# samson6460/tf2_YOLO

Hardware: AMD Instinct MI355X
Metric: images/sec training YOLOv3 416x416 bs=32/GPU (higher is better)
Workload: dtype f32-storage/fp16x2-mfma

## Files before the change

### include/yolo_hip.h

```cpp
#ifndef YOLO_HIP_H_
#define YOLO_HIP_H_

#include <stddef.h>
#include <stdint.h>

#ifdef __cplusplus
extern "C" {
#endif

typedef enum yolo_status {
  YOLO_OK = 0,
  YOLO_ERR_INVALID_ARG = -1,
  YOLO_ERR_LAUNCH = -2,
  YOLO_ERR_WORKSPACE = -3
} yolo_status;

enum { YOLO_ACT_LINEAR = 0, YOLO_ACT_LEAKY = 1, YOLO_ACT_MISH = 2 };
enum { YOLO_HEAD_V3 = 3, YOLO_HEAD_V2 = 2, YOLO_HEAD_V1 = 1, YOLO_HEAD_V4 = 4 };
enum { YOLO_NMS_HARD = 1, YOLO_NMS_SOFT = 2, YOLO_NMS_DIOU = 3 };

const char* yolo_last_error(void);
int yolo_abi_version(void);
int yolo_device_available(void);
int yolo_mfma_probe(const void* operands_f16, float* sink, int workgroups, int iters, double* flops_host, void* stream);

enum { YOLO_OPT_CONV_WIN = 0, YOLO_OPT_STAMPS = 1, YOLO_OPT_CONV_SK = 2, YOLO_OPT_CONV_PATCH = 5, YOLO_OPT_WGRAD_WIN = 6,
       YOLO_OPT_NMS_WALK = 7 ,
       YOLO_OPT_AB = 8  };
int yolo_set_option(int key, int value);
size_t yolo_conv_workspace_bytes(void);
int yolo_set_conv_workspace(void* p, size_t bytes, void* stream);
int yolo_set_debug_buffer(void* p, size_t bytes);

typedef struct yolo_conv_desc {
  int N, H, W, Cin;
  int Cout, kh, kw;
  int Ho, Wo;
  int sh, sw;
  int pad_t, pad_l;
} yolo_conv_desc;

#define YOLO_BN_STAT_SLOTS 64
// ... 246 lines not shown
```

### tf2_yolo_amd/csrc/conv.hip

```cpp
#include "conv_args.hpp"
#include <cstdlib>
#include <type_traits>

namespace yolo {

template <int BM, int BN, int WGM, int WGN, bool FLAT>
__global__ __launch_bounds__(256) void gather_conv_kernel(const GatherConvArgs a) {
  constexpr int BK = 32;
  constexpr int LD = BK + 4;
  constexpr int TM = BM / WGM / 32;
  constexpr int TN = BN / WGN / 32;
  constexpr int AR = BM / 32;
  constexpr int BR = BN / 32;
  static_assert(WGM * WGN == 4, "4 waves per block");
  static_assert(TM >= 1 && TN >= 1, "wave tile");

  extern __shared__ __attribute__((aligned(16))) float smem[];
  constexpr int BUF = (BM + BN) * LD;

  const int tid = threadIdx.x;
  const int lane = tid & 63;
  const int wave = tid >> 6;
  const int wm = wave / WGN, wn = wave % WGN;

// ... 1026 lines not shown
  int cap;
  unsigned* aux;
  int nslots;
};
static void set_bnred(GatherConvArgs& a, const BnRedArgs* b) {
  if (b == nullptr) return;
  a.bwd_y = b->y; a.bwd_scale = b->scale; a.bwd_shift = b->shift; a.bwd_mean = b->mean; a.bwd_invstd = b->invstd;
  a.bwd_act = b->act; a.bwd_part = b->part; a.bwd_cap = b->cap; a.bwd_aux = b->aux;
}

static int dgrad_impl(const yolo_conv_desc* d, const float* dy, const float* wT, float* dx, int accumulate,
                      void* stream, bool planes, BnRedArgs* bnred = nullptr) {
  if (int rc = validate_desc(d)) return rc;
  YOLO_REQUIRE(dy && wT && dx, "conv_dgrad: null pointer");
  const bool flat = (d->Cout % 32) != 0;
  YOLO_REQUIRE(!flat || (d->kh == 1 && d->kw == 1 && d->sh == 1 && d->sw == 1),
               "conv_dgrad: Cout %% 32 != 0 only supported for 1x1 stride-1 (head) convs");
  static const bool fuse_classes = env_int("YOLO_DGRAD_CLASSES", 1) != 0;
  if (planes && fuse_classes && d->sh * d->sw > 1 && d->sh * d->sw <= 4) {
    GatherConvArgs a{};
    a.src = dy;
    a.wgt = wT;
    a.dst = dx;
    a.N = d->N; a.Hs = d->Ho; a.Ws = d->Wo; a.Cs = d->Cout;
    a.sy = 1; a.sx = 1;
    a.Hd = d->H; a.Wd = d->W; a.Cd = d->Cin;
    a.osy = d->sh; a.osx = d->sw;
    a.Cout = d->Cin;
    a.ldw = d->kh * d->kw * d->Cout;
    a.accumulate = accumulate;
    a.kw = 1;
    int nt = 0, nc = 0;
    bool ok = true;
// ... 196 lines not shown
```

### tf2_yolo_amd/csrc/conv_args.hpp

```cpp
#pragma once
#include "common.hpp"

namespace yolo {

constexpr int MAX_TAPS = 49;

struct Tap {
  int oy, ox, woff;
};

struct ClassGeom {
  long long M;
  int Hg, Wg, ooy, oox, tap0, ntaps;
};

struct GatherConvArgs {
  const float* src;
  const float* wgt;
  const float* bias;
  float* dst;
  double* stats;
  unsigned* absmax;
  long long M;
  int N, Hs, Ws, Cs;
// ... 20 lines not shown
  const float* pl_pred;
  const unsigned* pl_in_bound;
  const unsigned* pl_res_bound;
  int pl_in_n, pl_res_n;
  unsigned* pl_out_words;
  float* head_y;
  const float* head_anchors;
  int head_A, head_C;
  int sk_grid;
  int tile_order;
  float* sk_slabs;
  unsigned* sk_tickets;
  int split_parts;
  int ncls;
  ClassGeom cls[4];
  unsigned long long* stamps;
  const float* bwd_y;
  const float* bwd_scale;
  const float* bwd_shift;
  const float* bwd_mean;
  const float* bwd_invstd;
  float* bwd_part;
  unsigned* bwd_aux;
  int bwd_act;
  int bwd_nslots;
  int bwd_cap;
  Tap taps[MAX_TAPS];
};

#define YOLO_BNRED_CHECK(a)                                                                                          \
// ... 40 lines not shown
                               void* planes, float* dst32, float* out_bound, hipStream_t st,
                               const int* bound_words = nullptr, const int* upsample = nullptr, int H = 0, int W = 0);
int launch_split_planes_padded(const float* x, long long rows, int Csrc, int C, void* planes, hipStream_t st);
int launch_split_planes_batch(const void* jobs, int njobs, long long total_blocks, hipStream_t st);
int launch_filter_transpose_batch(const void* jobs, int njobs, long long total_blocks, hipStream_t st);
int launch_gather_planes(GatherConvArgs& a, hipStream_t st);
bool conv_small_supported(const GatherConvArgs& a);
bool conv_small_head_supported(const GatherConvArgs& a);
int launch_conv_small(GatherConvArgs& a, hipStream_t st, int* nwg);
bool gather_planes_supported(const GatherConvArgs& a);
int conv_split_parts(const GatherConvArgs& a, long long nb, int bm, int min_cb, int idle_div);
int launch_split_reduce(GatherConvArgs& a, int bm, hipStream_t st);
float* conv_split_slabs();
int launch_conv_win(GatherConvArgs& a, int variant, hipStream_t st);
bool conv_win_supported(const GatherConvArgs& a);
enum { OPT_CONV_WIN = 0, OPT_STAMPS = 1, OPT_CONV_SK = 2, OPT_DBG = 3, OPT_TILE_ORDER = 4, OPT_CONV_PATCH = 5, OPT_WGRAD_WIN = 6, OPT_NMS_WALK = 7, OPT_EXP = 8, OPT_COUNT = 16 };
int set_conv_workspace(void* p, size_t bytes, hipStream_t st);
extern void* g_dbg_buf;
extern size_t g_dbg_bytes;
extern int g_opt[OPT_COUNT];
void init_options();
int launch_wgrad_planes(WgradArgs& a, hipStream_t st);
bool wgrad_planes_supported(const WgradArgs& a);
int launch_wgrad_win(WgradArgs& a, hipStream_t st);
bool wgrad_win_supported(const WgradArgs& a);
constexpr size_t WGRAD_WS_COLSUM_BYTES = 1 << 20;
void* wgrad_workspace(size_t* bytes);
bool stem_fwd_supported(const yolo_conv_desc* d);
struct StemEpiArgs {
  const float* scale;
  const float* shift;
// ... 23 lines not shown
```

### tf2_yolo_amd/csrc/conv_planes.hip

```cpp
#include "planes_epilogue.hpp"
#include <algorithm>
#include <cstdlib>
#include <type_traits>

namespace yolo {

__global__ __launch_bounds__(256) void planes_amax_kernel(const float* __restrict__ x, long long n4,
                                                         unsigned* __restrict__ header) {
  float m = 0.f;
  for (long long i = (long long)blockIdx.x * 256 + threadIdx.x; i < n4; i += (long long)gridDim.x * 256) {
    const f32x4 v = reinterpret_cast<const f32x4*>(x)[i];
    m = fmaxf(fmaxf(m, fmaxf(fabsf(v[0]), fabsf(v[1]))), fmaxf(fabsf(v[2]), fabsf(v[3])));
  }
#pragma unroll
  for (int o = 32; o > 0; o >>= 1) m = fmaxf(m, __shfl_xor(m, o, 64));
  __shared__ float wmax[4];
  if ((threadIdx.x & 63) == 0) wmax[threadIdx.x >> 6] = m;
  __syncthreads();
  if (threadIdx.x == 0) {
    m = fmaxf(fmaxf(wmax[0], wmax[1]), fmaxf(wmax[2], wmax[3]));
    if (__builtin_bit_cast(unsigned, m) > *reinterpret_cast<volatile unsigned*>(header))
      atomicMax(header, __builtin_bit_cast(unsigned, m));
  }
}
// ... 216 lines not shown
      if (g * 8 + 4 + j < Csrc) v1[j] = p[g * 8 + 4 + j];
    }
  }
  const Planes8 s = split8(v0, v1, sc);
  unsigned char* o = out + planes_unit_offset(row, g, C);
  *reinterpret_cast<u32x4*>(o) = s.h;
  *reinterpret_cast<u32x4*>(o + 512) = s.l;
}

constexpr int PF_KO_MASK = 31;
constexpr int PF_SPLIT = 32;
constexpr int PF_MULTI = 64;
constexpr int PF_DEEP1 = 128;
constexpr int PF_DEEP2 = 256;
constexpr int PF_BNRED = 512;
template <int BM, int BN, int WGM, int WGN, int FORM = 0>
__global__ __launch_bounds__(64 * WGM * WGN, (WGM * WGN >= 4 ? 2 : 1)) void gather_conv_planes_kernel(const GatherConvArgs a) {
  constexpr int NW = WGM * WGN;
  constexpr int TM = BM / WGM / 32;
  constexpr int TN = BN / WGN / 32;
  constexpr int RBA = BM / 32, RBB = BN / 32;
  constexpr int LPW = (RBA + RBB + NW - 1) / NW;
  static_assert(LPW <= 4, "loader layout: slot s = wave + i*NW loads A block s, or B block (s - RBA) % RBB");
  constexpr int ND = PL_PLANES * LPW;
  constexpr int STAGE_BYTES = (RBA + RBB) * PL_PLANES * 1024;
  constexpr int NBUF = 3 + ((FORM >> 7) & 3);

  extern __shared__ __attribute__((aligned(16))) unsigned char smem[];
  const unsigned lds_base = (unsigned)(size_t)smem;

  const int tid = threadIdx.x;
  const int lane = tid & 63;
  const int wave = __builtin_amdgcn_readfirstlane(tid >> 6);
  const int wm = wave / WGN, wn = wave % WGN;

  constexpr bool SPLIT = (FORM & PF_SPLIT) != 0;
  const int SP = SPLIT ? a.split_parts : 1;
  const int part = SPLIT ? (int)blockIdx.x / a.nblocks : 0;
  const int tile = xcd_remap(SPLIT ? (int)blockIdx.x - part * a.nblocks : (int)blockIdx.x, a.nblocks);
  constexpr bool MULTI = (FORM & PF_MULTI) != 0;
  constexpr bool BNRED = (FORM & PF_BNRED) != 0;
  const int tile_n = tile % a.tiles_n;
  const int cls = MULTI ? (tile / a.tiles_n) % a.ncls : 0;
  const int tile_m = MULTI ? tile / (a.tiles_n * a.ncls) : tile / a.tiles_n;
  const long long m0 = (long long)tile_m * BM;
  const int n0 = tile_n * BN;
  const EpiGeom G = MULTI ? EpiGeom{a.cls[cls].M, a.cls[cls].Hg, a.cls[cls].Wg, a.cls[cls].ooy, a.cls[cls].oox, 0, 0, 0,
                                    tile_m * a.ncls + cls + 1}
                          : epi_geom_of(a);
  const int tap0 = MULTI ? a.cls[cls].tap0 : 0;
  const int ntaps = MULTI ? a.cls[cls].ntaps : a.ntaps;
  if (MULTI && m0 >= G.M) {
    if (a.bwd_y != nullptr)
      for (int c = tid; c < BN; c += 64 * NW)
        if (n0 + c < a.Cout) {
          a.bwd_part[((long long)(G.slot1 - 1) * 2 + 0) * a.Cout + n0 + c] = 0.f;
// ... 18 lines not shown
#pragma unroll
  for (int i = 0; i < LPW; ++i) {
    const int slot = wave + i * NW;
    isA[i] = slot < RBA;
    const int rb = isA[i] ? slot : (slot - RBA) % RBB;
    nimg[i] = 0; ys0[i] = -(1 << 28); xs0[i] = 0; rowbaseB[i] = 0;
    if (isA[i]) {
      const long long m = m0 + rb * 32 + r;
      if (m < G.M) {
        nimg[i] = (int)(m / HgWg);
        const int rem = (int)(m - (long long)nimg[i] * HgWg);
        const int y = rem / G.Wg;
        ys0[i] = y * a.sy;
        xs0[i] = (rem - y * G.Wg) * a.sx;
      }
    } else {
      const int co = n0 + rb * 32 + r;
      const unsigned blk = co < a.Cout ? (unsigned)(co >> 4) : (unsigned)a.zero_blk_wgt;
      rowbaseB[i] = blk * blkstrideB + (co < a.Cout ? (co & 15) * 16 : 0) + hf * 256;
    }
    lds_mine[i] = lds_base + ((isA[i] ? 0 : RBA) + rb) * PL_PLANES * 1024;
    ld_voff[i] = 0; ld_soff[i] = 0;
  }

  int ld_tap = 0, ld_kk = 0, ld_cb = cb_lo;
  auto loader_tap = [&]() {
#pragma unroll
    for (int i = 0; i < LPW; ++i) {
      if (ld_cb >= cpt) {
        ld_voff[i] = isA[i] ? (unsigned)a.zero_blk_src * blkstrideA : (unsigned)a.zero_blk_wgt * blkstrideB;
        ld_soff[i] = 0;
      } else if (isA[i]) {
        const int ys = ys0[i] + a.taps[tap0 + ld_tap].oy, xs = xs0[i] + a.taps[tap0 + ld_tap].ox;
        const bool ok = ((unsigned)ys < (unsigned)a.Hs) && ((unsigned)xs < (unsigned)a.Ws);
        const int pix = (nimg[i] * a.Hs + ys) * a.Ws + xs;
        ld_voff[i] = (ok ? ((unsigned)pix >> 4) : (unsigned)a.zero_blk_src) * blkstrideA + (ok ? (pix & 15) * 16 : 0) + hf * 256;
        ld_soff[i] = (unsigned)ld_cb * PL_RECORD;
      } else {
        ld_voff[i] = rowbaseB[i];
        ld_soff[i] = (unsigned)((a.taps[tap0 + ld_tap].woff >> 4) + ld_cb) * PL_RECORD;
      }
    }
  };
  auto loader_next = [&]() {
#pragma unroll
    for (int i = 0; i < LPW; ++i) ld_soff[i] += PL_RECORD;
    const int kc_cur = (cpt - ld_cb < a.kc) ? (cpt - ld_cb) : a.kc;
    if (++ld_kk >= kc_cur) {
      ld_kk = 0;
      if (++ld_tap == ntaps) {
        ld_tap = 0;
        ld_cb += a.kc;
// ... 24 lines not shown

  f16x8 fa[2][PL_PLANES][TM], fb[2][PL_PLANES][TN];
  auto read_frags = [&](int buf, auto SET) {
    constexpr int S = decltype(SET)::value;
    const unsigned char* sb = smem + buf * STAGE_BYTES + lane * 16;
#pragma unroll
    for (int p = 0; p < PL_PLANES; ++p) {
#pragma unroll
      for (int i = 0; i < TM; ++i)
        fa[S][p][i] = *reinterpret_cast<const f16x8*>(sb + ((wm * TM + i) * PL_PLANES + p) * 1024);
#pragma unroll
      for (int j = 0; j < TN; ++j)
        fb[S][p][j] = *reinterpret_cast<const f16x8*>(sb + ((RBA + wn * TN + j) * PL_PLANES + p) * 1024);
    }
  };
  auto mfma_stage = [&](auto SET, int wbuf) {
    constexpr int S = decltype(SET)::value;
    constexpr int NM = TM * TN * 3;
#pragma unroll
    for (int q = 0; q < 3; ++q) {
      const int pa = (q == 0) ? 1 : 0;
      const int pb = (q == 1) ? 1 : 0;
#pragma unroll
      for (int i = 0; i < TM; ++i)
#pragma unroll
        for (int j = 0; j < TN; ++j) {
          if constexpr (!(FORM & 8)) acc[i][j] = __builtin_amdgcn_mfma_f32_32x32x16_f16(fa[S][pa][i], fb[S][pb][j], acc[i][j], 0, 0, 0);
          const int idx = (q * TM + i) * TN + j;
#pragma unroll
          for (int d = 0; d < ND; ++d)
            if (idx == (((d + 1) * NM) / (ND + 1) > 0 ? ((d + 1) * NM) / (ND + 1) - 1 : 0)) {
              __builtin_amdgcn_sched_barrier(0);
              if constexpr (!(FORM & 1)) issue_plane(d, wbuf);
              __builtin_amdgcn_sched_barrier(0);
            }
        }
    }
    loader_next();
  };

  using S0 = std::integral_constant<int, 0>;
  using S1 = std::integral_constant<int, 1>;
// ... 19 lines not shown
    for (; kt + 1 < nk; kt += 2) {
      step(rbuf, wbuf, S0{}, S1{});
      rbuf = (rbuf + 1 == NBUF) ? 0 : rbuf + 1;
      wbuf = (wbuf + 1 == NBUF) ? 0 : wbuf + 1;
      step(rbuf, wbuf, S1{}, S0{});
      rbuf = (rbuf + 1 == NBUF) ? 0 : rbuf + 1;
      wbuf = (wbuf + 1 == NBUF) ? 0 : wbuf + 1;
    }
    if (kt < nk) step(rbuf, wbuf, S0{}, S1{});
  }
  asm volatile("s_waitcnt vmcnt(0)" ::: "memory");
  __syncthreads();

  if constexpr (SPLIT)
    store_split_slab<TM, TN>(a, acc, BM * BN * 4, tile * SP + part, wave, lane);
  else if constexpr (MULTI)
    planes_epilogue<BM, BN, WGM, WGN, NBUF * STAGE_BYTES, 0, NoStamp, false, BNRED>(a, acc, smem, m0, n0, tile_m, wm, wn, lane, tid, NoStamp(), &G);
  else
    planes_epilogue<BM, BN, WGM, WGN, NBUF * STAGE_BYTES, (FORM & PF_KO_MASK), NoStamp, false, BNRED>(a, acc, smem, m0, n0, tile_m, wm, wn, lane, tid);
}

template <int BM, int BN, int WGM, int WGN, int FORM = 0>
static int launch_planes(GatherConvArgs& a, hipStream_t st) {
  const long long tiles_m = (a.M + BM - 1) / BM;
  a.tiles_n = (a.Cout + BN - 1) / BN;
  const long long nb = tiles_m * a.tiles_n;
  if (nb <= 0 || nb > 0x7fffffffLL) {
    set_error("conv(planes): bad grid %lld", nb);
    return YOLO_ERR_INVALID_ARG;
  }
// ... 23 lines not shown
  a.bwd_nslots = (int)tiles_m;
  YOLO_BNRED_CHECK(a)
  constexpr auto plain = &gather_conv_planes_kernel<BM, BN, WGM, WGN, FORM>;
  a.split_parts = 1;
  if constexpr (BM == 128 && BN == 128 && WGM == 2 && WGN == 2 && FORM == 0) {
    const int min_cb = a.ntaps >= 8 ? 1 : (8 + a.ntaps - 1) / a.ntaps;
    a.split_parts = conv_split_parts(a, nb, BM, min_cb, 4);
    if (a.split_parts > 1) {
      a.sk_slabs = conv_split_slabs();
      if (int rc = launch_lds<gather_conv_planes_kernel<BM, BN, WGM, WGN, PF_SPLIT>, lds>(
              dim3((unsigned)(nb * a.split_parts)), block, st, a, "gather_conv_planes_kernel(split)"))
        return rc;
      return launch_split_reduce(a, BM, st);
    }
  }
  if constexpr ((FORM & ~(PF_DEEP1 | PF_DEEP2)) == 0) {
    if (a.bwd_y != nullptr)
      return launch_lds<gather_conv_planes_kernel<BM, BN, WGM, WGN, FORM | PF_BNRED>, lds>(dim3((unsigned)nb), block, st, a,
                                                                                          "gather_conv_planes_kernel(bn reduce)");
  } else if (a.bwd_y != nullptr) {
    set_error("conv(planes): this diagnostic instantiation has no fused BatchNorm-backward reduction");
    return YOLO_ERR_INVALID_ARG;
  }
  return launch_lds<plain, lds>(dim3((unsigned)nb), block, st, a, "gather_conv_planes_kernel");
}

long long planes_bytes(long long rows, int C) { return planes_body_bytes(rows, C) + PL_HEADER; }

bool gather_planes_supported(const GatherConvArgs& a) { return (a.Cs % 16) == 0 && a.Cout >= 32; }

int launch_gather_planes(GatherConvArgs& a, hipStream_t st) {
  const long long rowsA = (long long)a.N * a.Hs * a.Ws;
  const long long bytesA = planes_bytes(rowsA, a.Cs), bytesB = planes_bytes(a.Cout, a.ldw);
  if (bytesA >= (1LL << 32) || bytesB >= (1LL << 32)) {
    set_error("conv(planes): operand planes exceed 4 GiB (%lld, %lld bytes)", bytesA, bytesB);
    return YOLO_ERR_INVALID_ARG;
  }
  a.src_bytes = (unsigned)bytesA;
  a.wgt_bytes = (unsigned)bytesB;
  a.zero_blk_src = (int)((rowsA + 15) / 16);
  a.zero_blk_wgt = (a.Cout + 15) / 16;
  static const int nt = env_int("YOLO_NT_STORE", 1);
  a.nt_store = nt;
  static const int vecst = env_int("YOLO_VEC_STORE", 1);
  a.vec_store = vecst;
  static const int dbg = env_int("YOLO_PLANES_DBG", 0);
  a.dbg = dbg;
  static const int kc_env = env_int("YOLO_PLANES_KC", 0);
  a.kc = kc_env > 0 ? kc_env : (a.Cs >> 4);
  if (a.kc > (a.Cs >> 4)) a.kc = a.Cs >> 4;
  init_options();
  if (g_opt[OPT_CONV_WIN] != 0 && a.ncls <= 1) {
    const int rc = launch_conv_win(a, g_opt[OPT_CONV_WIN], st);
    if (rc <= 0) return rc;
  }
  static const int deep_env = env_int("YOLO_PLANES_DEEP", -1);
  const int deep = deep_env >= 0 ? deep_env : (a.Cout <= 64 ? 1 : 2);
  if (deep && a.ntaps == 1 && a.ncls <= 1) {
    if (a.Cout <= 32) return deep == 1 ? launch_planes<128, 32, 4, 1, PF_DEEP1>(a, st) : launch_planes<128, 32, 4, 1, PF_DEEP2>(a, st);
    if (a.Cout <= 64) return deep == 1 ? launch_planes<128, 64, 4, 2, PF_DEEP1>(a, st) : launch_planes<128, 64, 4, 2, PF_DEEP2>(a, st);
  }
  if (a.Cout <= 32) return launch_planes<128, 32, 4, 1>(a, st);
  if (a.Cout <= 64) return launch_planes<128, 64, 4, 2>(a, st);
  static const int narrow_below = env_int("YOLO_PLANES_NARROW_BELOW", 0);
  if (((a.M + 127) / 128) * ((a.Cout + 127) / 128) < narrow_below) return launch_planes<128, 64, 4, 2>(a, st);
  static const int waves_env = env_int("YOLO_PLANES_WAVES", 0);
// ... 284 lines not shown
```

### tf2_yolo_amd/csrc/planes_epilogue.hpp

```cpp
#pragma once
#include "planes.hpp"
#include "act.hpp"

namespace yolo {

struct NoStamp {
  __device__ __forceinline__ void operator()(int) const {}
};

struct EpiGeom {
  long long M;
  int Hg, Wg, ooy, oox;
  int pn, py0, px0;
  int slot1;
};
__device__ __forceinline__ EpiGeom epi_geom_of(const GatherConvArgs& a) {
  return EpiGeom{a.M, a.Hg, a.Wg, a.ooy, a.oox, 0, 0, 0, 0};
}

template <int TM, int TN>
__device__ __forceinline__ void store_split_slab(const GatherConvArgs& a, f32x16 (&acc)[TM][TN], const int slab_bytes,
                                                 const int slab, const int wave, const int lane) {
  unsigned char* mine = reinterpret_cast<unsigned char*>(a.sk_slabs) + (size_t)slab * slab_bytes;
  const __amdgpu_buffer_rsrc_t rs = __builtin_amdgcn_make_buffer_rsrc(mine, 0, slab_bytes, 0x00020000);
#pragma unroll
  for (int i = 0; i < TM; ++i)
#pragma unroll
    for (int j = 0; j < TN; ++j)
#pragma unroll
      for (int q4 = 0; q4 < 4; ++q4) {
        const f32x4 f = {acc[i][j][4 * q4], acc[i][j][4 * q4 + 1], acc[i][j][4 * q4 + 2], acc[i][j][4 * q4 + 3]};
        __builtin_amdgcn_raw_buffer_store_b128(__builtin_bit_cast(u32x4, f), rs,
                                               (((wave * TM + i) * TN + j) * 4 + q4) * 1024 + lane * 16, 0, 0);
      }
}

template <int BM, int BN, int WGM, int WGN, int LDS_BYTES, int DBG = 0, class STAMP = NoStamp, bool PATCH = false, bool BNRED = false>
__device__ __forceinline__ void planes_epilogue(const GatherConvArgs& a, f32x16 (&acc)[BM / WGM / 32][BN / WGN / 32],
                                                unsigned char* smem, const long long m0, const int n0, const int tile_m,
                                                const int wm, const int wn, const int lane, const int tid,
                                                const STAMP& stampf = STAMP(), const EpiGeom* geom = nullptr) {
  const EpiGeom G = geom != nullptr ? *geom : epi_geom_of(a);
  constexpr int NT = 64 * WGM * WGN;
  constexpr int NW = WGM * WGN;
  constexpr int TM = BM / WGM / 32;
  constexpr int TN = BN / WGN / 32;
  const int wave = wm * WGN + wn;
  float* smf = reinterpret_cast<float*>(smem);
  long long* rowoff = reinterpret_cast<long long*>(smf);
  const bool dense = a.osy == 1 && a.osx == 1 && G.ooy == 0 && G.oox == 0 && a.Hd == G.Hg && a.Wd == G.Wg;
  {
    const int HgWg = G.Hg * G.Wg;
    for (int rr = tid; rr < BM; rr += NT) {
      const long long m = m0 + rr;
      long long off = -1;
      if constexpr (PATCH) {
        const int y = G.py0 + (rr >> 4), x = G.px0 + (rr & 15);
        if (y < G.Hg && x < G.Wg) off = (((long long)G.pn * a.Hd + y) * a.Wd + x) * a.Cd;
      } else if (m < G.M) {
        if (dense) {
          off = m * a.Cd;
        } else {
          const int n = (int)(m / HgWg);
          const int rem = (int)(m - (long long)n * HgWg);
          const int y = rem / G.Wg;
          const int x = rem - y * G.Wg;
          off = (((long long)n * a.Hd + (y * a.osy + G.ooy)) * a.Wd + (x * a.osx + G.oox)) * a.Cd;
        }
      }
      rowoff[rr] = off;
    }
  }
  __syncthreads();
  stampf(0);

  const float unscale =
      reinterpret_cast<const float*>(reinterpret_cast<const unsigned char*>(a.src) + a.src_bytes - PL_HEADER)[2] *
      reinterpret_cast<const float*>(reinterpret_cast<const unsigned char*>(a.wgt) + a.wgt_bytes - PL_HEADER)[2];
  float* sred = smf + 2 * BM;
  float csum[TN], csq[TN], cmx[TN];
#pragma unroll
  for (int j = 0; j < TN; ++j) csum[j] = csq[j] = cmx[j] = 0.f;
  [[maybe_unused]] float bs1[TN], bs2[TN];
#pragma unroll
  for (int j = 0; j < TN; ++j) bs1[j] = bs2[j] = 0.f;
  asm volatile("" ::"v"(unscale));
  stampf(1);
  const int rows_valid = PATCH ? BM : ((G.M - m0 < (long long)BM) ? (int)(G.M - m0) : BM);
  const bool want_stats = a.stats != nullptr || a.absmax != nullptr;
  [[maybe_unused]] unsigned long long rowmask = ~0ull;
  if constexpr (PATCH) {
    static_assert(BM / WGM / 32 <= 4, "row mask: at most 4 row blocks per wave");
    rowmask = 0;
    if (want_stats) {
#pragma unroll
      for (int i = 0; i < BM / WGM / 32; ++i)
#pragma unroll
        for (int q = 0; q < 16; ++q)
          if (rowoff[(wm * (BM / WGM / 32) + i) * 32 + (q & 3) + 8 * (q >> 2) + 4 * (lane >> 5)] >= 0)
            rowmask |= 1ull << (i * 16 + q);
    }
  }
  const bool bnred = BNRED && a.bwd_y != nullptr && a.stats == nullptr;
  float bn_mx = 0.f;
  constexpr int WCOLS = TN * 32;
  constexpr int TLD = WCOLS + 4;
  constexpr int FIXED = 2 * BM + WGM * BN * 3;
  constexpr int RP = ((FIXED + NW * 32 * TLD) * 4 <= LDS_BYTES) ? 32 : 16;
  constexpr bool VEC_OK = (FIXED + NW * RP * TLD) * 4 <= LDS_BYTES && (RP * WCOLS / 4) % 64 == 0;
  const bool vec = VEC_OK && a.vec_store && (a.Cout & 3) == 0 && (a.Cd & 3) == 0 && !(a.accumulate && a.stats != nullptr) &&
                   (DBG & 16) == 0;
  if constexpr (VEC_OK) {
  if (vec) {
    float* strip = smf + FIXED + wave * (RP * TLD);
    constexpr int C4 = WCOLS / 4;
    constexpr int ITER = RP * C4 / 64;
    static_assert(64 % C4 == 0, "store loop: a lane keeps its four columns");
    const int bcol = n0 + wn * WCOLS + (lane % C4) * 4;
    f32x4 b_sc = {0.f, 0.f, 0.f, 0.f}, b_sh = b_sc, b_mu = b_sc, b_iv = b_sc, b_s1 = b_sc, b_s2 = b_sc;
    constexpr int NPASS = TM * (32 / RP);
    constexpr bool PRE_OLD = TM * TN <= 2;
    [[maybe_unused]] f32x4 ypre[BNRED ? NPASS : 1][BNRED ? ITER : 1];
    [[maybe_unused]] f32x4 opre[BNRED && PRE_OLD ? NPASS : 1][BNRED && PRE_OLD ? ITER : 1];
    if constexpr (BNRED)
// ... 98 lines not shown
                const f32x4 yv = ypre[ps][h0 + k];
#pragma unroll
                for (int e = 0; e < 4; ++e) {
                  const float dz = v[e] * act_grad(fmaf(b_sc[e], yv[e], b_sh[e]), a.bwd_act);
                  b_s1[e] += dz;
                  b_s2[e] = fmaf(dz, (yv[e] - b_mu[e]) * b_iv[e], b_s2[e]);
                  bn_mx = fmaxf(bn_mx, fabsf(dz));
                }
              }
            }
          }
          }
        } else {
        long long offs[ITER];
        f32x4 vv[ITER];
#pragma unroll
        for (int it = 0; it < ITER; ++it) {
          const int idx = lane + it * 64;
          const int rl = idx / C4, c4 = idx - rl * C4;
          offs[it] = rowoff[row0 + rl];
          vv[it] = *reinterpret_cast<const f32x4*>(strip + rl * TLD + c4 * 4);
        }
#pragma unroll
        for (int it = 0; it < ITER; ++it) {
          const int idx = lane + it * 64;
          const int c4 = idx % C4;
          const int col = n0 + wn * WCOLS + c4 * 4;
          if (offs[it] >= 0 && col < a.Cout) {
            f32x4* p = reinterpret_cast<f32x4*>(a.dst + offs[it] + col);
            f32x4 v = vv[it];
            if (a.epi_res != nullptr) v += *reinterpret_cast<const f32x4*>(a.epi_res + offs[it] + col);
            if (a.accumulate) v += *p;
            if (a.nt_store) __builtin_nontemporal_store(v, p); else *p = v;
          }
        }
        }
        asm volatile("s_waitcnt lgkmcnt(0)" ::: "memory");
      }
    }
    if (bnred) {
#pragma unroll
      for (int o = C4; o < 64; o <<= 1)
#pragma unroll
        for (int e = 0; e < 4; ++e) {
          b_s1[e] += __shfl_xor(b_s1[e], o, 64);
          b_s2[e] += __shfl_xor(b_s2[e], o, 64);
// ... 7 lines not shown
      }
    }
    stampf(2);
  }
  }
  if (!vec) {
#pragma unroll
    for (int i = 0; i < TM; ++i) {
      long long offs[16];
#pragma unroll
      for (int q = 0; q < 16; ++q) offs[q] = rowoff[(wm * TM + i) * 32 + (q & 3) + 8 * (q >> 2) + 4 * (lane >> 5)];
#pragma unroll
      for (int j = 0; j < TN; ++j) {
        const int col = n0 + (wn * TN + j) * 32 + (lane & 31);
        const bool cok = col < a.Cout;
        const float bv = (a.bias != nullptr && cok) ? a.bias[col] : 0.f;
        const float esc = (a.epi_scale != nullptr && cok) ? a.epi_scale[col] : 1.f;
        const float esh = (a.epi_scale != nullptr && cok) ? a.epi_shift[col] : 0.f;
        const float rsc = (bnred && cok) ? a.bwd_scale[col] : 0.f, rsh = (bnred && cok) ? a.bwd_shift[col] : 0.f;
        const float rmu = (bnred && cok) ? a.bwd_mean[col] : 0.f, riv = (bnred && cok) ? a.bwd_invstd[col] : 0.f;
#pragma unroll
        for (int q = 0; q < 16; ++q) {
          const bool ok = cok && offs[q] >= 0;
          float v = fmaf(acc[i][j][q], unscale, bv);
          if (a.epi_scale != nullptr) v = act_fwd(fmaf(esc, v, esh), a.epi_act);
          const float vstat = v;
          if (ok) {
            if (a.epi_res != nullptr) v += a.epi_res[offs[q] + col];
            if (a.accumulate) v += a.dst[offs[q] + col];
            if constexpr ((DBG & 16) != 0) { if (v == 1234.5678f) a.dst[offs[q] + col] = v; }
            else if (a.nt_store && !bnred) __builtin_nontemporal_store(v, &a.dst[offs[q] + col]); else a.dst[offs[q] + col] = v;
            if (bnred) {
              const float yv = a.bwd_y[offs[q] + col];
              const float dz = v * act_grad(fmaf(rsc, yv, rsh), a.bwd_act);
              bs1[j] += dz;
              bs2[j] = fmaf(dz, (yv - rmu) * riv, bs2[j]);
              bn_mx = fmaxf(bn_mx, fabsf(dz));
            }
          }
          const float vm = ok ? (a.epi_scale != nullptr ? vstat : v) : 0.f;
          csum[j] += vm;
          csq[j] = fmaf(vm, vm, csq[j]);
          cmx[j] = fmaxf(cmx[j], fabsf(vm));
        }
      }
    }
  }
  if (bnred) {
// ... 72 lines not shown
```

### tf2_yolo_amd/csrc/runtime.hip

```cpp
#include "conv_args.hpp"
#include <cstdlib>
#include <cstring>

namespace yolo {

static thread_local char g_err[512] = "";

void set_error(const char* fmt, ...) {
  va_list ap;
  va_start(ap, fmt);
  vsnprintf(g_err, sizeof(g_err), fmt, ap);
  va_end(ap);
}

int g_opt[OPT_COUNT];
void* g_dbg_buf = nullptr;
size_t g_dbg_bytes = 0;
static void options_from_env() {
  for (int i = 0; i < OPT_COUNT; ++i) g_opt[i] = 0;
  g_opt[OPT_CONV_WIN] = env_int("YOLO_CONV_WIN", 1);
  g_opt[OPT_CONV_SK] = env_int("YOLO_CONV_SK", 1);
  g_opt[OPT_CONV_PATCH] = env_int("YOLO_CONV_PATCH", 1);
  g_opt[OPT_WGRAD_WIN] = env_int("YOLO_WGRAD_WIN", 1);
  g_opt[OPT_NMS_WALK] = env_int("YOLO_NMS_WALK", 0);
  g_opt[OPT_EXP] = env_int("YOLO_EXP", 0);
}
void init_options() {
  static bool done = false;
  if (done) return;
  done = true;
  options_from_env();
}

}

extern "C" int yolo_set_option(int key, int value) {
  yolo::init_options();
  if (key == -1) {
    yolo::options_from_env();
    return YOLO_OK;
// ... 62 lines not shown
```

### tf2_yolo_amd/ops.py

```python
import ctypes
from ctypes import byref, c_void_p

import torch

from . import _lib
from . import tape as _tape
from ._lib import ConvDesc, LossCfg, YoloHipError, check

BN_EPS = 1e-3
BN_MOMENTUM = 0.99
BN_STAT_SLOTS = 64
BN_RED_SLOTS = 512
SPLIT_BATCH_UNITS = 4


class KernelTimer:

    def __init__(self):
        self.pending = []

    def bracket(self, name, flops, launches, fn, layer=None):
        s, e = torch.cuda.Event(enable_timing=True), torch.cuda.Event(enable_timing=True)
        s.record()
        fn()
# ... 80 lines not shown
        if CONV_PATCH == 2 or ((narrow or ws > 64) and tiles >= 256):
            return "conv_patch_planes_kernel<%s>" % ("256,64" if narrow else "128,128")
    if win is not None and CONV_WIN and cout >= 128:
        ws, m = win[:2]
        wgm = CONV_WIN if CONV_WIN in (2, 4) else (0 if ws > 64 else 2)
        if wgm:
            return "conv_win_planes_kernel<%d,128>" % (64 * wgm)
    if cout <= 32:
        return "gather_conv_planes_kernel<128,32,4,1>"
    if cout <= 64:
        return "gather_conv_planes_kernel<128,64,4,2>"
    waves8 = _PLANES_WAVES == 8 or (_PLANES_WAVES == 0 and k1)
    return "gather_conv_planes_kernel<128,128,%s>" % ("4,2" if waves8 else "2,2")


def _win_key(d, hs, ws, cs):
    if d.kh == 3 and d.kw == 3 and d.sh == 1 and d.sw == 1 and d.pad_t == 1 and d.pad_l == 1 and cs % 16 == 0 \
            and d.H == d.Ho and d.W == d.Wo:
        return (ws, d.N * hs * ws, hs, d.N)
    return None


def _gather_variant(cout, flat, m=None):
    bn = 32 if cout <= 32 else (64 if cout <= 64 else 128)
    bm = 128
    if bn == 128 and not flat and m is not None and ((m + 127) // 128) * ((cout + 127) // 128) <= 512:
        bm = 64
    if CONV_MODE == "split" and not flat and cout > 32:
        waves = {(128, 64): "2,2", (64, 128): "1,4", (128, 128): "4,2"}[(bm, bn)]
        return f"gather_conv_split_kernel<{bm},{bn},{waves}>"
    return f"gather_conv_kernel<{bm},{bn}{',flat' if flat else ''}>"


OPT_CONV_WIN = 0
OPT_CONV_SK = 2
OPT_CONV_PATCH = 5
OPT_WGRAD_WIN = 6
OPT_NMS_WALK = 7
_CONV_WS = None


def ensure_conv_workspace():
    global _CONV_WS
    if _CONV_WS is not None and _CONV_WS.device.index != torch.cuda.current_device():
        raise YoloHipError(f"libyolo_hip.so was initialised on cuda:{_CONV_WS.device.index} and cannot also serve "
                           f"cuda:{torch.cuda.current_device()}: start one process per GPU")
    if _CONV_WS is None:
        lib = _lib.load()
        n = int(lib.yolo_conv_workspace_bytes())
        _CONV_WS = torch.empty(n, dtype=torch.uint8, device="cuda")
        check(lib.yolo_set_conv_workspace(_p(_CONV_WS), n, _stream()), "yolo_set_conv_workspace")
    return _CONV_WS

# ... 58 lines not shown
                              "will run them one after the other (create_side_streams() earlier, or raise GPU_MAX_HW_QUEUES)")
            _SIDE_STREAMS[(dev, role)] = st
            _first_use(st, dev)
    return {role: _SIDE_STREAMS[(dev, role)] for role in ("wgrad", "comm")}


def concurrent_stream(role, beside=None, device=None):
    st = create_side_streams(device)[role]
    want = torch.cuda.current_device() if device is None else torch.device(device).index
    if want is not None and st.device.index != want:
        raise YoloHipError(f"side stream of role {role!r} lives on cuda:{st.device.index}, not on cuda:{want}")
    return st


def set_option(key, value):
    global WGRAD_WIN
    check(_lib.load().yolo_set_option(int(key), int(value)), "yolo_set_option")
    if int(key) == OPT_WGRAD_WIN:
        WGRAD_WIN = int(value)


def reset_options():
    global WGRAD_WIN
    check(_lib.load().yolo_set_option(-1, 0), "yolo_set_option")
    WGRAD_WIN = int(_os.environ.get("YOLO_WGRAD_WIN", "1"))


def _stream():
    return c_void_p(torch.cuda.current_stream().cuda_stream)


def _p(t):
    if t is None:
        return c_void_p(0)
    if _tape.ACTIVE is not None:
        _tape.ACTIVE.keep.append(t)
    return c_void_p(t.data_ptr())


def _chk_f32(*ts):
# ... 313 lines not shown
        if (b.y.numel() != dx.numel() or min(t.numel() for t in (b.scale, b.shift, b.mean, b.invstd)) < d.Cin
                or b.partials.numel() < b.cap * 2 * d.Cin or b.aux is None or b.aux.numel() < 68):
            raise YoloHipError("conv2d_dgrad_planes: the fused reduction's buffers do not match the descriptor")
    def run():
        if bnred is None:
            check(_lib.load().yolo_conv2d_dgrad_planes(byref(d), _p(dyp), _p(wTp), _p(dx), int(bool(accumulate)), _stream()),
                  "yolo_conv2d_dgrad_planes")
            return
        n = ctypes.c_int(0)
        check(_lib.load().yolo_conv2d_dgrad_planes_bnred(byref(d), _p(dyp), _p(wTp), _p(dx), int(bool(accumulate)), _p(b.y),
                                                         _p(b.scale), _p(b.shift), _p(b.mean), _p(b.invstd), int(b.act),
                                                         _p(b.partials), int(b.cap), _p(b.aux), byref(n), _stream()),
              "yolo_conv2d_dgrad_planes_bnred")
        b.nslots = n.value
    if TIMER is not None:
        TIMER.bracket(_planes_variant(d.Cin, _win_key(d, d.Ho, d.Wo, d.Cout), d.kh * d.kw == 1 and d.sh * d.sw == 1), _conv_flops(d), 1, run,
                      _layer_key(d, "dgrad"))
    else:
        run()
    return dx


def conv2d_wgrad_planes(d, xp, dyp, dw, dy=None, dbias=None):
    _chk_f32(dw, dy, dbias)
    if dw.numel() != d.Cout * d.kh * d.kw * d.Cin:
        raise YoloHipError("conv2d_wgrad_planes: dw size does not match the descriptor")
    if xp.numel() < planes_bytes(d.N * d.H * d.W, d.Cin) or dyp.numel() < planes_bytes(d.N * d.Ho * d.Wo, d.Cout):
        raise YoloHipError("conv2d_wgrad_planes: planes buffers do not match the descriptor")
    def run():
        check(_lib.load().yolo_conv2d_wgrad_planes(byref(d), _p(xp), _p(dyp), _p(dw), _stream()),
              "yolo_conv2d_wgrad_planes")
    if TIMER is not None:
# ... 578 lines not shown
```

Baseline: 1081.

## Pack four output-parity classes into one 128-column tile for Cin=32 dgrad

For data-gradient convolutions with only 32 input channels, the four 2x2 output-parity classes are stacked as four 32-wide column groups of one 128-column MFMA tile. Each class gets its own weight-offset table per source tap, and the epilogue uses four row-offset tables to scatter results back to the interleaved output pixels. This is meant to fill the otherwise mostly-empty N dimension of the tile and read dy once for all classes. A default skip mask avoids MFMAs on class/tap pairs with no weight. The cost is extra epilogue address work and extra LDS for the tables.

```diff
diff --git a/include/yolo_hip.h b/include/yolo_hip.h
--- a/include/yolo_hip.h
+++ b/include/yolo_hip.h
@@ -26,6 +26,7 @@
 
 enum { YOLO_OPT_CONV_WIN = 0, YOLO_OPT_STAMPS = 1, YOLO_OPT_CONV_SK = 2, YOLO_OPT_CONV_PATCH = 5, YOLO_OPT_WGRAD_WIN = 6,
        YOLO_OPT_NMS_WALK = 7 ,
+       YOLO_OPT_DGRAD_COLS = 9,
        YOLO_OPT_AB = 8  };
 int yolo_set_option(int key, int value);
 size_t yolo_conv_workspace_bytes(void);
diff --git a/tf2_yolo_amd/csrc/conv.hip b/tf2_yolo_amd/csrc/conv.hip
--- a/tf2_yolo_amd/csrc/conv.hip
+++ b/tf2_yolo_amd/csrc/conv.hip
@@ -1,4 +1,5 @@
 #include "conv_args.hpp"
+#include "dgrad_cols_plan.hpp"
 #include <cstdlib>
 #include <type_traits>
 
@@ -1064,9 +1065,41 @@
   if (int rc = validate_desc(d)) return rc;
   YOLO_REQUIRE(dy && wT && dx, "conv_dgrad: null pointer");
   const bool flat = (d->Cout % 32) != 0;
-  YOLO_REQUIRE(!flat || (d->kh == 1 && d->kw == 1 && d->sh == 1 && d->sw == 1),
+  YOLO_REQUIRE(planes || !flat || (d->kh == 1 && d->kw == 1 && d->sh == 1 && d->sw == 1),
                "conv_dgrad: Cout %% 32 != 0 only supported for 1x1 stride-1 (head) convs");
   static const bool fuse_classes = env_int("YOLO_DGRAD_CLASSES", 1) != 0;
+  init_options();
+  if (planes && bnred == nullptr && g_opt[OPT_DGRAD_COLS] != 0 && d->Cin == 32 && d->Cout % 16 == 0 && d->kh * d->kw <= 9) {
+    const int o = g_opt[OPT_DGRAD_COLS];
+    const bool strided = d->sh * d->sw > 1;
+    const bool want = strided ? (o & 1) != 0 : (d->kh * d->kw > 1 ? (o & 2) != 0 : (o & 8) != 0);
+    DgradColsPlan pl;
+    if (want && dgrad_cols_plan(d, &pl)) {
+      GatherConvArgs a{};
+      a.src = dy;
+      a.wgt = wT;
+      a.dst = dx;
+      a.N = d->N; a.Hs = d->Ho; a.Ws = d->Wo; a.Cs = d->Cout;
+      a.Hg = pl.Hg; a.Wg = pl.Wg;
+      a.sy = pl.step_y; a.sx = pl.step_x;
+      a.Hd = d->H; a.Wd = d->W; a.Cd = d->Cin;
+      a.osy = 2; a.osx = 2;
+      a.cols = d->Cin;
+      a.cols_dense = (o & 4) != 0;
+      a.Cout = DGC_CLASSES * d->Cin;
+      a.ldw = d->kh * d->kw * d->Cout;
+      a.accumulate = accumulate;
+      a.kw = 1;
+      a.M = (long long)d->N * pl.Hg * pl.Wg;
+      a.ntaps = pl.ntaps;
+      for (int t = 0; t < pl.ntaps; ++t) {
+        a.taps[t] = Tap{pl.oy[t], pl.ox[t], 0};
+        for (int q = 0; q < DGC_CLASSES; ++q) a.cwoff[t][q] = pl.woff[t][q];
+      }
+      a.cmask = pl.used;
+      return launch_gather_planes(a, as_stream(stream));
+    }
+  }
   if (planes && fuse_classes && d->sh * d->sw > 1 && d->sh * d->sw <= 4) {
     GatherConvArgs a{};
     a.src = dy;
diff --git a/tf2_yolo_amd/csrc/conv_args.hpp b/tf2_yolo_amd/csrc/conv_args.hpp
--- a/tf2_yolo_amd/csrc/conv_args.hpp
+++ b/tf2_yolo_amd/csrc/conv_args.hpp
@@ -58,6 +58,9 @@
   int split_parts;
   int ncls;
   ClassGeom cls[4];
+  int cols, cols_dense;
+  int cwoff[16][4];
+  unsigned long long cmask;
   unsigned long long* stamps;
   const float* bwd_y;
   const float* bwd_scale;
@@ -128,7 +131,7 @@
 float* conv_split_slabs();
 int launch_conv_win(GatherConvArgs& a, int variant, hipStream_t st);
 bool conv_win_supported(const GatherConvArgs& a);
-enum { OPT_CONV_WIN = 0, OPT_STAMPS = 1, OPT_CONV_SK = 2, OPT_DBG = 3, OPT_TILE_ORDER = 4, OPT_CONV_PATCH = 5, OPT_WGRAD_WIN = 6, OPT_NMS_WALK = 7, OPT_EXP = 8, OPT_COUNT = 16 };
+enum { OPT_CONV_WIN = 0, OPT_STAMPS = 1, OPT_CONV_SK = 2, OPT_DBG = 3, OPT_TILE_ORDER = 4, OPT_CONV_PATCH = 5, OPT_WGRAD_WIN = 6, OPT_NMS_WALK = 7, OPT_EXP = 8, OPT_DGRAD_COLS = 9, OPT_COUNT = 16 };
 int set_conv_workspace(void* p, size_t bytes, hipStream_t st);
 extern void* g_dbg_buf;
 extern size_t g_dbg_bytes;
diff --git a/tf2_yolo_amd/csrc/conv_planes.hip b/tf2_yolo_amd/csrc/conv_planes.hip
--- a/tf2_yolo_amd/csrc/conv_planes.hip
+++ b/tf2_yolo_amd/csrc/conv_planes.hip
@@ -254,6 +254,8 @@
 constexpr int PF_DEEP1 = 128;
 constexpr int PF_DEEP2 = 256;
 constexpr int PF_BNRED = 512;
+constexpr int PF_COLS = 1024;
+constexpr int PF_COLSKIP = 2048;
 template <int BM, int BN, int WGM, int WGN, int FORM = 0>
 __global__ __launch_bounds__(64 * WGM * WGN, (WGM * WGN >= 4 ? 2 : 1)) void gather_conv_planes_kernel(const GatherConvArgs a) {
   constexpr int NW = WGM * WGN;
@@ -280,6 +282,9 @@
   const int tile = xcd_remap(SPLIT ? (int)blockIdx.x - part * a.nblocks : (int)blockIdx.x, a.nblocks);
   constexpr bool MULTI = (FORM & PF_MULTI) != 0;
   constexpr bool BNRED = (FORM & PF_BNRED) != 0;
+  constexpr bool COLS = (FORM & PF_COLS) != 0;
+  constexpr bool COLSKIP = (FORM & PF_COLSKIP) != 0;
+  static_assert(!COLS || (BN == 128 && RBB == 4 && !MULTI && !SPLIT && !BNRED), "class columns: one 128-column tile, four classes");
   const int tile_n = tile % a.tiles_n;
   const int cls = MULTI ? (tile / a.tiles_n) % a.ncls : 0;
   const int tile_m = MULTI ? tile / (a.tiles_n * a.ncls) : tile / a.tiles_n;
@@ -328,6 +333,8 @@
         ys0[i] = y * a.sy;
         xs0[i] = (rem - y * G.Wg) * a.sx;
       }
+    } else if constexpr (COLS) {
+      rowbaseB[i] = (unsigned)(r >> 4) * blkstrideB + (r & 15) * 16 + hf * 256;
     } else {
       const int co = n0 + rb * 32 + r;
       const unsigned blk = co < a.Cout ? (unsigned)(co >> 4) : (unsigned)a.zero_blk_wgt;
@@ -350,6 +357,10 @@
         const int pix = (nimg[i] * a.Hs + ys) * a.Ws + xs;
         ld_voff[i] = (ok ? ((unsigned)pix >> 4) : (unsigned)a.zero_blk_src) * blkstrideA + (ok ? (pix & 15) * 16 : 0) + hf * 256;
         ld_soff[i] = (unsigned)ld_cb * PL_RECORD;
+      } else if constexpr (COLS) {
+        const int wo = a.cwoff[ld_tap][(wave + i * NW - RBA) % RBB];
+        ld_voff[i] = wo >= 0 ? rowbaseB[i] : (unsigned)a.zero_blk_wgt * blkstrideB;
+        ld_soff[i] = wo >= 0 ? (unsigned)((wo >> 4) + ld_cb) * PL_RECORD : 0u;
       } else {
         ld_voff[i] = rowbaseB[i];
         ld_soff[i] = (unsigned)((a.taps[tap0 + ld_tap].woff >> 4) + ld_cb) * PL_RECORD;
@@ -404,9 +415,22 @@
         fb[S][p][j] = *reinterpret_cast<const f16x8*>(sb + ((RBA + wn * TN + j) * PL_PLANES + p) * 1024);
     }
   };
+  [[maybe_unused]] int cs_tap = 0, cs_kk = 0, cs_cb = cb_lo;
   auto mfma_stage = [&](auto SET, int wbuf) {
     constexpr int S = decltype(SET)::value;
     constexpr int NM = TM * TN * 3;
+    [[maybe_unused]] unsigned use = ~0u;
+    if constexpr (COLSKIP) {
+      use = __builtin_amdgcn_readfirstlane((unsigned)(a.cmask >> (cs_tap * 4 + wn * TN)));
+      const int kc_cur = (cpt - cs_cb < a.kc) ? (cpt - cs_cb) : a.kc;
+      if (++cs_kk >= kc_cur) {
+        cs_kk = 0;
+        if (++cs_tap == ntaps) {
+          cs_tap = 0;
+          cs_cb += a.kc;
+        }
+      }
+    }
 #pragma unroll
     for (int q = 0; q < 3; ++q) {
       const int pa = (q == 0) ? 1 : 0;
@@ -415,7 +439,9 @@
       for (int i = 0; i < TM; ++i)
 #pragma unroll
         for (int j = 0; j < TN; ++j) {
-          if constexpr (!(FORM & 8)) acc[i][j] = __builtin_amdgcn_mfma_f32_32x32x16_f16(fa[S][pa][i], fb[S][pb][j], acc[i][j], 0, 0, 0);
+          if constexpr (COLSKIP) {
+            if ((use >> j) & 1) acc[i][j] = __builtin_amdgcn_mfma_f32_32x32x16_f16(fa[S][pa][i], fb[S][pb][j], acc[i][j], 0, 0, 0);
+          } else if constexpr (!(FORM & 8)) acc[i][j] = __builtin_amdgcn_mfma_f32_32x32x16_f16(fa[S][pa][i], fb[S][pb][j], acc[i][j], 0, 0, 0);
           const int idx = (q * TM + i) * TN + j;
 #pragma unroll
           for (int d = 0; d < ND; ++d)
@@ -465,6 +491,8 @@
 
   if constexpr (SPLIT)
     store_split_slab<TM, TN>(a, acc, BM * BN * 4, tile * SP + part, wave, lane);
+  else if constexpr (COLS)
+    planes_epilogue<BM, BN, WGM, WGN, NBUF * STAGE_BYTES, 0, NoStamp, false, false, true>(a, acc, smem, m0, n0, tile_m, wm, wn, lane, tid);
   else if constexpr (MULTI)
     planes_epilogue<BM, BN, WGM, WGN, NBUF * STAGE_BYTES, 0, NoStamp, false, BNRED>(a, acc, smem, m0, n0, tile_m, wm, wn, lane, tid, NoStamp(), &G);
   else
@@ -518,7 +546,13 @@
       return launch_split_reduce(a, BM, st);
     }
   }
-  if constexpr ((FORM & ~(PF_DEEP1 | PF_DEEP2)) == 0) {
+  if constexpr ((FORM & PF_COLS) != 0) {
+    if (a.bwd_y != nullptr || a.stats != nullptr || a.cols != 32 || a.Cout != 4 * a.cols || a.Cd != a.cols || a.ntaps > 16) {
+      set_error("conv(planes, class columns): needs 32 channels, at most 16 source taps, no fused reduction or statistics");
+      return YOLO_ERR_INVALID_ARG;
+    }
+    return launch_lds<plain, lds>(dim3((unsigned)nb), block, st, a, "gather_conv_planes_kernel(class columns)");
+  } else if constexpr ((FORM & ~(PF_DEEP1 | PF_DEEP2)) == 0) {
     if (a.bwd_y != nullptr)
       return launch_lds<gather_conv_planes_kernel<BM, BN, WGM, WGN, FORM | PF_BNRED>, lds>(dim3((unsigned)nb), block, st, a,
                                                                                           "gather_conv_planes_kernel(bn reduce)");
@@ -535,7 +569,8 @@
 
 int launch_gather_planes(GatherConvArgs& a, hipStream_t st) {
   const long long rowsA = (long long)a.N * a.Hs * a.Ws;
-  const long long bytesA = planes_bytes(rowsA, a.Cs), bytesB = planes_bytes(a.Cout, a.ldw);
+  const int wrows = a.cols > 0 ? a.cols : a.Cout;
+  const long long bytesA = planes_bytes(rowsA, a.Cs), bytesB = planes_bytes(wrows, a.ldw);
   if (bytesA >= (1LL << 32) || bytesB >= (1LL << 32)) {
     set_error("conv(planes): operand planes exceed 4 GiB (%lld, %lld bytes)", bytesA, bytesB);
     return YOLO_ERR_INVALID_ARG;
@@ -543,7 +578,7 @@
   a.src_bytes = (unsigned)bytesA;
   a.wgt_bytes = (unsigned)bytesB;
   a.zero_blk_src = (int)((rowsA + 15) / 16);
-  a.zero_blk_wgt = (a.Cout + 15) / 16;
+  a.zero_blk_wgt = (wrows + 15) / 16;
   static const int nt = env_int("YOLO_NT_STORE", 1);
   a.nt_store = nt;
   static const int vecst = env_int("YOLO_VEC_STORE", 1);
@@ -554,6 +589,8 @@
   a.kc = kc_env > 0 ? kc_env : (a.Cs >> 4);
   if (a.kc > (a.Cs >> 4)) a.kc = a.Cs >> 4;
   init_options();
+  if (a.cols > 0)
+    return a.cols_dense ? launch_planes<128, 128, 2, 2, PF_COLS>(a, st) : launch_planes<128, 128, 2, 2, PF_COLS | PF_COLSKIP>(a, st);
   if (g_opt[OPT_CONV_WIN] != 0 && a.ncls <= 1) {
     const int rc = launch_conv_win(a, g_opt[OPT_CONV_WIN], st);
     if (rc <= 0) return rc;
diff --git a/tf2_yolo_amd/csrc/dgrad_cols_plan.hpp b/tf2_yolo_amd/csrc/dgrad_cols_plan.hpp
--- /dev/null
+++ b/tf2_yolo_amd/csrc/dgrad_cols_plan.hpp
@@ -0,0 +1,69 @@
+#pragma once
+#include "../../include/yolo_hip.h"
+
+namespace yolo {
+
+constexpr int DGC_MAX_TAPS = 16;
+constexpr int DGC_CLASSES = 4;
+
+struct DgradColsPlan {
+  int Hg, Wg;
+  int step_y, step_x;
+  int ntaps;
+  int oy[DGC_MAX_TAPS], ox[DGC_MAX_TAPS];
+  int woff[DGC_MAX_TAPS][DGC_CLASSES];
+  unsigned long long used;
+};
+
+inline bool dgrad_cols_plan(const yolo_conv_desc* d, DgradColsPlan* p) {
+  if ((d->sh != 1 && d->sh != 2) || (d->sw != 1 && d->sw != 2) || d->kh <= 0 || d->kw <= 0 || d->H <= 0 || d->W <= 0)
+    return false;
+  p->Hg = (d->H + 1) / 2;
+  p->Wg = (d->W + 1) / 2;
+  p->step_y = 2 / d->sh;
+  p->step_x = 2 / d->sw;
+  p->ntaps = 0;
+  p->used = 0;
+  int ylo = 1 << 30, yhi = -(1 << 30), xlo = 1 << 30, xhi = -(1 << 30);
+  for (int py = 0; py < 2; ++py)
+    for (int r = 0; r < d->kh; ++r) {
+      const int t = py + d->pad_t - r;
+      if (((t % d->sh) + d->sh) % d->sh != 0) continue;
+      const int o = t / d->sh;
+      ylo = o < ylo ? o : ylo;
+      yhi = o > yhi ? o : yhi;
+    }
+  for (int px = 0; px < 2; ++px)
+    for (int s = 0; s < d->kw; ++s) {
+      const int t = px + d->pad_l - s;
+      if (((t % d->sw) + d->sw) % d->sw != 0) continue;
+      const int o = t / d->sw;
+      xlo = o < xlo ? o : xlo;
+      xhi = o > xhi ? o : xhi;
+    }
+  if (ylo > yhi || xlo > xhi) return false;
+  if ((long long)(yhi - ylo + 1) * (xhi - xlo + 1) > DGC_MAX_TAPS) return false;
+  for (int oy = yhi; oy >= ylo; --oy)
+    for (int ox = xhi; ox >= xlo; --ox) {
+      int w[DGC_CLASSES];
+      bool any = false;
+      for (int py = 0; py < 2; ++py)
+        for (int px = 0; px < 2; ++px) {
+          const int r = py + d->pad_t - oy * d->sh, s = px + d->pad_l - ox * d->sw;
+          const bool ok = r >= 0 && r < d->kh && s >= 0 && s < d->kw;
+          w[py * 2 + px] = ok ? (r * d->kw + s) * d->Cout : -1;
+          any = any || ok;
+        }
+      if (!any) continue;
+      const int t = p->ntaps++;
+      p->oy[t] = oy;
+      p->ox[t] = ox;
+      for (int q = 0; q < DGC_CLASSES; ++q) {
+        p->woff[t][q] = w[q];
+        if (w[q] >= 0) p->used |= 1ull << (t * DGC_CLASSES + q);
+      }
+    }
+  return p->ntaps > 0;
+}
+
+}
diff --git a/tf2_yolo_amd/csrc/planes_epilogue.hpp b/tf2_yolo_amd/csrc/planes_epilogue.hpp
--- a/tf2_yolo_amd/csrc/planes_epilogue.hpp
+++ b/tf2_yolo_amd/csrc/planes_epilogue.hpp
@@ -35,7 +35,8 @@
       }
 }
 
-template <int BM, int BN, int WGM, int WGN, int LDS_BYTES, int DBG = 0, class STAMP = NoStamp, bool PATCH = false, bool BNRED = false>
+template <int BM, int BN, int WGM, int WGN, int LDS_BYTES, int DBG = 0, class STAMP = NoStamp, bool PATCH = false, bool BNRED = false,
+          bool COLS = false>
 __device__ __forceinline__ void planes_epilogue(const GatherConvArgs& a, f32x16 (&acc)[BM / WGM / 32][BN / WGN / 32],
                                                 unsigned char* smem, const long long m0, const int n0, const int tile_m,
                                                 const int wm, const int wn, const int lane, const int tid,
@@ -48,9 +49,26 @@
   const int wave = wm * WGN + wn;
   float* smf = reinterpret_cast<float*>(smem);
   long long* rowoff = reinterpret_cast<long long*>(smf);
+  static_assert(!COLS || (!PATCH && !BNRED), "class columns: plain data gradients only");
+  constexpr int NTAB = COLS ? 4 : 1;
   const bool dense = a.osy == 1 && a.osx == 1 && G.ooy == 0 && G.oox == 0 && a.Hd == G.Hg && a.Wd == G.Wg;
   {
     const int HgWg = G.Hg * G.Wg;
+    if constexpr (COLS) {
+      for (int e = tid; e < NTAB * BM; e += NT) {
+        const int q = e / BM;
+        const long long m = m0 + (e - q * BM);
+        long long off = -1;
+        if (m < G.M) {
+          const int n = (int)(m / HgWg);
+          const int rem = (int)(m - (long long)n * HgWg);
+          const int yb = rem / G.Wg;
+          const int y = 2 * yb + (q >> 1), x = 2 * (rem - yb * G.Wg) + (q & 1);
+          if (y < a.Hd && x < a.Wd) off = (((long long)n * a.Hd + y) * a.Wd + x) * a.Cd;
+        }
+        rowoff[e] = off;
+      }
+    } else
     for (int rr = tid; rr < BM; rr += NT) {
       const long long m = m0 + rr;
       long long off = -1;
@@ -77,7 +95,7 @@
   const float unscale =
       reinterpret_cast<const float*>(reinterpret_cast<const unsigned char*>(a.src) + a.src_bytes - PL_HEADER)[2] *
       reinterpret_cast<const float*>(reinterpret_cast<const unsigned char*>(a.wgt) + a.wgt_bytes - PL_HEADER)[2];
-  float* sred = smf + 2 * BM;
+  float* sred = smf + 2 * NTAB * BM;
   float csum[TN], csq[TN], cmx[TN];
 #pragma unroll
   for (int j = 0; j < TN; ++j) csum[j] = csq[j] = cmx[j] = 0.f;
@@ -105,9 +123,10 @@
   float bn_mx = 0.f;
   constexpr int WCOLS = TN * 32;
   constexpr int TLD = WCOLS + 4;
-  constexpr int FIXED = 2 * BM + WGM * BN * 3;
+  constexpr int FIXED = 2 * NTAB * BM + WGM * BN * 3;
   constexpr int RP = ((FIXED + NW * 32 * TLD) * 4 <= LDS_BYTES) ? 32 : 16;
   constexpr bool VEC_OK = (FIXED + NW * RP * TLD) * 4 <= LDS_BYTES && (RP * WCOLS / 4) % 64 == 0;
+  static_assert(!COLS || (VEC_OK && RP == 32 && LDS_BYTES <= 48 * 1024), "class columns: four tables, 32-row passes, inside 48 KB");
   const bool vec = VEC_OK && a.vec_store && (a.Cout & 3) == 0 && (a.Cd & 3) == 0 && !(a.accumulate && a.stats != nullptr) &&
                    (DBG & 16) == 0;
   if constexpr (VEC_OK) {
@@ -236,11 +255,13 @@
         } else {
         long long offs[ITER];
         f32x4 vv[ITER];
+        [[maybe_unused]] const int ccol = wn * WCOLS + (lane % C4) * 4;
+        [[maybe_unused]] const int cq = COLS ? ccol / a.cols : 0;
 #pragma unroll
         for (int it = 0; it < ITER; ++it) {
           const int idx = lane + it * 64;
           const int rl = idx / C4, c4 = idx - rl * C4;
-          offs[it] = rowoff[row0 + rl];
+          offs[it] = rowoff[(COLS ? cq * BM : 0) + row0 + rl];
           vv[it] = *reinterpret_cast<const f32x4*>(strip + rl * TLD + c4 * 4);
         }
 #pragma unroll
@@ -248,10 +269,11 @@
           const int idx = lane + it * 64;
           const int c4 = idx % C4;
           const int col = n0 + wn * WCOLS + c4 * 4;
+          const int dcol = COLS ? col - cq * a.cols : col;
           if (offs[it] >= 0 && col < a.Cout) {
-            f32x4* p = reinterpret_cast<f32x4*>(a.dst + offs[it] + col);
+            f32x4* p = reinterpret_cast<f32x4*>(a.dst + offs[it] + dcol);
             f32x4 v = vv[it];
-            if (a.epi_res != nullptr) v += *reinterpret_cast<const f32x4*>(a.epi_res + offs[it] + col);
+            if (a.epi_res != nullptr) v += *reinterpret_cast<const f32x4*>(a.epi_res + offs[it] + dcol);
             if (a.accumulate) v += *p;
             if (a.nt_store) __builtin_nontemporal_store(v, p); else *p = v;
           }
@@ -289,6 +311,13 @@
       for (int j = 0; j < TN; ++j) {
         const int col = n0 + (wn * TN + j) * 32 + (lane & 31);
         const bool cok = col < a.Cout;
+        [[maybe_unused]] int dcol = col;
+        if constexpr (COLS) {
+          const int cq = col / a.cols;
+          dcol = col - cq * a.cols;
+#pragma unroll
+          for (int q = 0; q < 16; ++q) offs[q] = rowoff[cq * BM + (wm * TM + i) * 32 + (q & 3) + 8 * (q >> 2) + 4 * (lane >> 5)];
+        }
         const float bv = (a.bias != nullptr && cok) ? a.bias[col] : 0.f;
         const float esc = (a.epi_scale != nullptr && cok) ? a.epi_scale[col] : 1.f;
         const float esh = (a.epi_scale != nullptr && cok) ? a.epi_shift[col] : 0.f;
@@ -301,12 +330,12 @@
           if (a.epi_scale != nullptr) v = act_fwd(fmaf(esc, v, esh), a.epi_act);
           const float vstat = v;
           if (ok) {
-            if (a.epi_res != nullptr) v += a.epi_res[offs[q] + col];
-            if (a.accumulate) v += a.dst[offs[q] + col];
-            if constexpr ((DBG & 16) != 0) { if (v == 1234.5678f) a.dst[offs[q] + col] = v; }
-            else if (a.nt_store && !bnred) __builtin_nontemporal_store(v, &a.dst[offs[q] + col]); else a.dst[offs[q] + col] = v;
+            if (a.epi_res != nullptr) v += a.epi_res[offs[q] + dcol];
+            if (a.accumulate) v += a.dst[offs[q] + dcol];
+            if constexpr ((DBG & 16) != 0) { if (v == 1234.5678f) a.dst[offs[q] + dcol] = v; }
+            else if (a.nt_store && !bnred) __builtin_nontemporal_store(v, &a.dst[offs[q] + dcol]); else a.dst[offs[q] + dcol] = v;
             if (bnred) {
-              const float yv = a.bwd_y[offs[q] + col];
+              const float yv = a.bwd_y[offs[q] + dcol];
               const float dz = v * act_grad(fmaf(rsc, yv, rsh), a.bwd_act);
               bs1[j] += dz;
               bs2[j] = fmaf(dz, (yv - rmu) * riv, bs2[j]);
diff --git a/tf2_yolo_amd/csrc/runtime.hip b/tf2_yolo_amd/csrc/runtime.hip
--- a/tf2_yolo_amd/csrc/runtime.hip
+++ b/tf2_yolo_amd/csrc/runtime.hip
@@ -24,6 +24,7 @@
   g_opt[OPT_WGRAD_WIN] = env_int("YOLO_WGRAD_WIN", 1);
   g_opt[OPT_NMS_WALK] = env_int("YOLO_NMS_WALK", 0);
   g_opt[OPT_EXP] = env_int("YOLO_EXP", 0);
+  g_opt[OPT_DGRAD_COLS] = env_int("YOLO_DGRAD_COLS", 1);
 }
 void init_options() {
   static bool done = false;
diff --git a/tf2_yolo_amd/ops.py b/tf2_yolo_amd/ops.py
--- a/tf2_yolo_amd/ops.py
+++ b/tf2_yolo_amd/ops.py
@@ -118,6 +118,14 @@
     return "gather_conv_planes_kernel<128,128,%s>" % ("4,2" if waves8 else "2,2")
 
 
+def _dgrad_cols_covers(d, bnred):
+    if bnred is not None or d.Cin != 32 or d.Cout % 16 or d.kh * d.kw > 9:
+        return False
+    if d.sh * d.sw > 1:
+        return bool(DGRAD_COLS & 1)
+    return bool(DGRAD_COLS & (2 if d.kh * d.kw > 1 else 8))
+
+
 def _win_key(d, hs, ws, cs):
     if d.kh == 3 and d.kw == 3 and d.sh == 1 and d.sw == 1 and d.pad_t == 1 and d.pad_l == 1 and cs % 16 == 0 \
             and d.H == d.Ho and d.W == d.Wo:
@@ -141,6 +149,8 @@
 OPT_CONV_PATCH = 5
 OPT_WGRAD_WIN = 6
 OPT_NMS_WALK = 7
+OPT_DGRAD_COLS = 9
+DGRAD_COLS = int(_os.environ.get("YOLO_DGRAD_COLS", "1"))
 _CONV_WS = None
 
 
@@ -229,16 +239,19 @@
 
 
 def set_option(key, value):
-    global WGRAD_WIN
+    global WGRAD_WIN, DGRAD_COLS
     check(_lib.load().yolo_set_option(int(key), int(value)), "yolo_set_option")
     if int(key) == OPT_WGRAD_WIN:
         WGRAD_WIN = int(value)
+    if int(key) == OPT_DGRAD_COLS:
+        DGRAD_COLS = int(value)
 
 
 def reset_options():
-    global WGRAD_WIN
+    global WGRAD_WIN, DGRAD_COLS
     check(_lib.load().yolo_set_option(-1, 0), "yolo_set_option")
     WGRAD_WIN = int(_os.environ.get("YOLO_WGRAD_WIN", "1"))
+    DGRAD_COLS = int(_os.environ.get("YOLO_DGRAD_COLS", "1"))
 
 
 def _stream():
@@ -582,8 +595,9 @@
               "yolo_conv2d_dgrad_planes_bnred")
         b.nslots = n.value
     if TIMER is not None:
-        TIMER.bracket(_planes_variant(d.Cin, _win_key(d, d.Ho, d.Wo, d.Cout), d.kh * d.kw == 1 and d.sh * d.sw == 1), _conv_flops(d), 1, run,
-                      _layer_key(d, "dgrad"))
+        name = ("gather_conv_planes_kernel<128,128,2,2,cols>" if _dgrad_cols_covers(d, bnred) else
+                _planes_variant(d.Cin, _win_key(d, d.Ho, d.Wo, d.Cout), d.kh * d.kw == 1 and d.sh * d.sw == 1))
+        TIMER.bracket(name, _conv_flops(d), 1, run, _layer_key(d, "dgrad"))
     else:
         run()
     return dx
```

After: 1081, median of 3. Within noise of the previous version (+0.0%).
